# BuTTerK3ks/AA-RMVSNet

Hardware: AMD Instinct MI355X
Metric: depth-hypotheses/sec (ref-views x H x W x D / s) (higher is better)
Workload: dtype fp32-class split-fp16 (3 products: cells, deconvs, omega conv on f16 MFMA, lo*lo dropped, fp32 accumulate; fp32 elsewhere); 1 GPU; dtu_eval_1600x1184_n7_d512; ref_views_per_gpu=1, views=7, H=1184, W=1600, D=512, global_batch=1, parallelism=ref-view shard x1

## Files before the change

aa-rmvsnet_amd/csrc/warp_cost.hip:

```cpp
#include <hip/hip_runtime.h>

#include <cfloat>
#include <climits>
#include <cstdlib>
#include <cstring>

#include "device_common.h"

namespace aarmvs {

__device__ __forceinline__ void sample_pos(const float* __restrict__ m, float depth, float x,
                                           float y, int H, int W, float& ix, float& iy) {
  float p[3];
#pragma unroll
  for (int k = 0; k < 3; ++k) {
    const float rx = __fadd_rn(__fadd_rn(__fmul_rn(m[4 * k + 0], x), __fmul_rn(m[4 * k + 1], y)),
                               m[4 * k + 2]);
    p[k] = __fadd_rn(__fmul_rn(rx, depth), m[4 * k + 3]);
  }
  float z = p[2];
  if (z == 0.0f) z = __fadd_rn(z, 1e-4f);
  const float px = __fdiv_rn(p[0], z), py = __fdiv_rn(p[1], z);
  const float gx = __fsub_rn(__fdiv_rn(px, (float)(W - 1) * 0.5f), 1.0f);
  const float gy = __fsub_rn(__fdiv_rn(py, (float)(H - 1) * 0.5f), 1.0f);
// ... 238 lines not shown
__device__ __forceinline__ void gn_relu4(const float (&x)[4], const GnStat& s, const float* gw,
                                         const float* gb, bool relu, float (&y)[4]) {
#pragma unroll
  for (int c = 0; c < 4; ++c) {
    const float sc = s.rstd * gw[c];
    const float sh = gb[c] - s.mean * sc;
    const float v = x[c] * sc + sh;
    y[c] = relu ? fmaxf(v, 0.0f) : v;
  }
}

__device__ __forceinline__ void conv1x1_4(const float (&x)[4], const float* w, const float* bias,
                                          float (&y)[4]) {
#pragma unroll
  for (int co = 0; co < 4; ++co) {
    float s = 0.f;
#pragma unroll
    for (int ci = 0; ci < 4; ++ci) s = fmaf(w[co * 4 + ci], x[ci], s);
    y[co] = s + bias[co];
  }
}

__device__ __forceinline__ float omega_weight(const float4 q, const GnStat* gs, const OmegaP& o) {
  const float t[4] = {q.x, q.y, q.z, q.w};
  float aa[4], t2[4], bb[4], t3[4], g3[4];
  gn_relu4(t, gs[0], o.g0w, o.g0b, true, aa);
  conv1x1_4(aa, o.w1, o.b1, t2);
  gn_relu4(t2, gs[1], o.g1w, o.g1b, true, bb);
  conv1x1_4(bb, o.w2, o.b2, t3);
  gn_relu4(t3, gs[2], o.g2w, o.g2b, false, g3);
  float s = 0.f;
#pragma unroll
  for (int c = 0; c < 4; ++c) s = fmaf(o.wo[c], fmaxf(g3[c] + aa[c], 0.0f), s);
  return sigmoidf_(s + o.bo);
}

__device__ __forceinline__ size_t st_index(int b, int v, int k, int nsrc) {
  return (((size_t)b * nsrc + v) * 3 + k) * kSlots * 2;
}

constexpr int kTileW = 32, kTileH = 16, kTileThreads = kTileW * kTileH;
constexpr int kTileWaves = kTileThreads / 64;

__device__ __forceinline__ int xcd_tile(int bid, int nb) {
  const int q8 = nb >> 3, r8 = nb & 7, xcd = bid & 7;
  return (xcd < r8 ? xcd * (q8 + 1) : r8 * (q8 + 1) + (xcd - r8) * q8) + (bid >> 3);
}

struct TapF {
  float xf, yf;
  float wt[4];
};

__device__ __forceinline__ TapF tap_f(const float* __restrict__ m, float dep, int x, int y, int H,
                                      int W) {
  float ix, iy;
  sample_pos(m, dep, (float)x, (float)y, H, W, ix, iy);
  TapF t;
  t.xf = floorf(ix);
  t.yf = floorf(iy);
  const float wx = __fsub_rn(ix, t.xf), wy = __fsub_rn(iy, t.yf);
  const float ex = __fsub_rn(1.0f, wx), sy = __fsub_rn(1.0f, wy);
  t.wt[0] = __fmul_rn(sy, ex);
  t.wt[1] = __fmul_rn(sy, wx);
  t.wt[2] = __fmul_rn(wy, ex);
  t.wt[3] = __fmul_rn(wy, wx);
  return t;
}

__device__ __forceinline__ void box_extend(const TapF& t, int H, int W, int& lx, int& ly, int& hx,
                                           int& hy) {
  if (!(t.xf == t.xf) || !(t.yf == t.yf)) return;
  const float xl = fmaxf(t.xf, 0.f), xh = fminf(t.xf + 1.f, (float)(W - 1));
  const float yl = fmaxf(t.yf, 0.f), yh = fminf(t.yf + 1.f, (float)(H - 1));
  if (xl <= xh && yl <= yh) {
    lx = min(lx, (int)xl);
    hx = max(hx, (int)xh);
    ly = min(ly, (int)yl);
    hy = max(hy, (int)yh);
  }
}

struct Box {
  int x0, y0, nx, ny;
};

template <int NW = kTileWaves>
__device__ __forceinline__ Box box_reduce(int lx, int ly, int hx, int hy, int (*red)[4]) {
  const int lane = threadIdx.x & 63, wave = threadIdx.x >> 6;
  auto mn = [](int a, int b) { return min(a, b); };
  auto mx = [](int a, int b) { return max(a, b); };
  lx = wave_reduce_i32(lx, INT_MAX, mn);
  ly = wave_reduce_i32(ly, INT_MAX, mn);
  hx = wave_reduce_i32(hx, INT_MIN, mx);
  hy = wave_reduce_i32(hy, INT_MIN, mx);
  if (lane == 0) {
    red[wave][0] = lx;
    red[wave][1] = ly;
    red[wave][2] = hx;
    red[wave][3] = hy;
  }
  __syncthreads();
#pragma unroll
  for (int w = 0; w < NW; ++w) {
    lx = min(lx, red[w][0]);
    ly = min(ly, red[w][1]);
    hx = max(hx, red[w][2]);
    hy = max(hy, red[w][3]);
  }
  Box bx;
  bx.x0 = __builtin_amdgcn_readfirstlane(lx);
  bx.y0 = __builtin_amdgcn_readfirstlane(ly);
  bx.nx = __builtin_amdgcn_readfirstlane(hx >= lx ? hx - lx + 1 : 0);
  bx.ny = __builtin_amdgcn_readfirstlane(hy >= ly ? hy - ly + 1 : 0);
  return bx;
}

__device__ __forceinline__ uint32_t box_magic(int nx) {
  return nx > 1 ? 0xFFFFFFFFu / (uint32_t)nx + 1u : 0u;
}
__device__ __forceinline__ int box_row(int p, int nx, uint32_t mg) {
  return nx > 1 ? (int)__umulhi((uint32_t)p, mg) : p;
}

struct TapP {
  uint32_t pix[4];
  float wt[4];
};

__device__ __forceinline__ TapP tap_p(const TapF& t, bool valid, int H, int W, bool lds,
                                      const Box& bx, uint32_t zpix) {
  TapP o;
#pragma unroll
  for (int k = 0; k < 4; ++k) {
    o.wt[k] = t.wt[k];
    const float xf = t.xf + (float)(k & 1), yf = t.yf + (float)(k >> 1);
    const bool ok = valid && (xf > -1.0f) && (xf < (float)W) && (yf > -1.0f) && (yf < (float)H);
    const int xi = ok ? (int)xf : bx.x0, yi = ok ? (int)yf : bx.y0;
    const uint32_t p = lds ? __umul24((uint32_t)(yi - bx.y0), (uint32_t)bx.nx) + (uint32_t)(xi - bx.x0)
                           : __umul24((uint32_t)yi, (uint32_t)W) + (uint32_t)xi;
    o.pix[k] = ok ? p : zpix;
  }
  return o;
}

__device__ __forceinline__ TapP tap_p4(const TapF& t, bool valid, int H, int W, bool lds,
                                      const Box& bx, uint32_t zpix) {
  TapP o;
#pragma unroll
  for (int k = 0; k < 4; ++k) o.wt[k] = t.wt[k];
  const float xf1 = t.xf + 1.0f, yf1 = t.yf + 1.0f;
  const bool cx0 = t.xf > -1.0f && t.xf < (float)W, cx1 = xf1 > -1.0f && xf1 < (float)W;
  const bool cy0 = valid && t.yf > -1.0f && t.yf < (float)H;
  const bool cy1 = valid && yf1 > -1.0f && yf1 < (float)H;
  const int ox = lds ? bx.x0 : 0, oy = lds ? bx.y0 : 0, rs = lds ? bx.nx : W;
  const int p00 = __mul24((int)t.yf - oy, rs) + ((int)t.xf - ox);
  o.pix[0] = cy0 && cx0 ? (uint32_t)p00 : zpix;
  o.pix[1] = cy0 && cx1 ? (uint32_t)(p00 + 1) : zpix;
  o.pix[2] = cy1 && cx0 ? (uint32_t)(p00 + rs) : zpix;
  o.pix[3] = cy1 && cx1 ? (uint32_t)(p00 + rs + 1) : zpix;
  return o;
}

__device__ __forceinline__ float bil1(float v0, float v1, float v2, float v3, const TapP& t) {
  return __fmaf_rn(v3, t.wt[3], __fmaf_rn(v2, t.wt[2], __fmaf_rn(v1, t.wt[1], __fmul_rn(v0, t.wt[0]))));
}

__device__ __forceinline__ float4 bil4(float4 v0, float4 v1, float4 v2, float4 v3, const TapP& t) {
  return make_float4(bil1(v0.x, v1.x, v2.x, v3.x, t), bil1(v0.y, v1.y, v2.y, v3.y, t),
                     bil1(v0.z, v1.z, v2.z, v3.z, t), bil1(v0.w, v1.w, v2.w, v3.w, t));
}

__device__ __forceinline__ float4 sqdiff4(float4 g, float4 r) {
  const float dx = __fsub_rn(g.x, r.x), dy = __fsub_rn(g.y, r.y);
  const float dz = __fsub_rn(g.z, r.z), dw = __fsub_rn(g.w, r.w);
  return make_float4(__fmul_rn(dx, dx), __fmul_rn(dy, dy), __fmul_rn(dz, dz), __fmul_rn(dw, dw));
}

__device__ __forceinline__ float4 ld_c8(__amdgpu_buffer_rsrc_t r, uint32_t p, int s, int HW) {
  return ld4(r, (uint32_t)(s >> 1) * (uint32_t)HW * 32u + p * 32u + 16u * (uint32_t)(s & 1));
}

__device__ __forceinline__ float swap_pair(float v) {
  return __int_as_float(__builtin_amdgcn_mov_dpp(__float_as_int(v), 0xB1, 0xF, 0xF, false));
}
__device__ __forceinline__ void sample_pos_pair(const float* __restrict__ m, float depth, float x,
                                                float y, int H, int W, int h, float& ix,
                                                float& iy) {
  auto row = [&](int k) {
    const float rx = __fadd_rn(__fadd_rn(__fmul_rn(m[4 * k + 0], x), __fmul_rn(m[4 * k + 1], y)),
                               m[4 * k + 2]);
    return __fadd_rn(__fmul_rn(rx, depth), m[4 * k + 3]);
  };
  const float ph = h ? row(1) : row(0);
  float z = row(2);
  if (z == 0.0f) z = __fadd_rn(z, 1e-4f);
  const int dim = h ? H : W;
  const float g = __fsub_rn(__fdiv_rn(__fdiv_rn(ph, z), (float)(dim - 1) * 0.5f), 1.0f);
  const float i = __fmaf_rn(__fadd_rn(g, 1.0f), (float)dim * 0.5f, -0.5f);
  const float o = swap_pair(i);
  ix = h ? o : i;
  iy = h ? i : o;
}

constexpr int kXRows = 4;
template <int XV = 0, int XR = kXRows>
__global__ void __launch_bounds__(2 * XR * kTileW)
__attribute__((amdgpu_waves_per_eu((XV & 8) ? 6 : (XV & 4) ? 5 : 4))) cost_x_kernel(PipeArgs a,
                                                              const float* __restrict__ P,
                                                              const float* __restrict__ Rel) {
  __shared__ GnStat gs[AARMVS_MAX_SRC][3];
  const int tid = threadIdx.x, b = blockIdx.y;
  const int H = a.H, W = a.W, HW = H * W, nsrc = a.nsrc;
  const int seq = xcd_tile(blockIdx.x, gridDim.x);
  const int tile = seq / a.npl, kp = seq - tile * a.npl;
  const int tiles_x = (W + kTileW - 1) / kTileW;
  const int h = tid & 1, q = tid >> 1;
  const int gy = (tile / tiles_x) * XR + q / kTileW, gx = (tile % tiles_x) * kTileW + q % kTileW;
  if (tid < 3 * nsrc) {
    const int v = tid / 3, k = tid % 3;
    gs[v][k] = stat_read(a.st_prev + kp * a.st_kstride + st_index(b, v, k, nsrc), 4.0 * HW);
  }
  __syncthreads();
  if (gy >= H || gx >= W) return;
  const float4* __restrict__ t1p = a.t1_prev + kp * a.t1_kstride;
  float* const omega_out = kp == a.omega_k ? a.omega_out : nullptr;
  OmegaP o;
  load_omega(a, P, o);
  const float dep = a.dvals[b * a.D + a.d_prev + kp];
  const uint32_t fbytes = (uint32_t)((size_t)kC * HW * 4);
  const __amdgpu_buffer_rsrc_t rref = uniform_rsrc(a.ref + (size_t)b * kC * HW, fbytes);
  const size_t p = (size_t)gy * W + gx;
  float4 rf[4];
#pragma unroll
  for (int c = 0; c < 4; ++c) rf[c] = ld_c8(rref, (uint32_t)p, 2 * c + h, HW);
  float acc[16];
#pragma unroll
  for (int j = 0; j < 16; ++j) acc[j] = 0.f;
  float wv[AARMVS_MAX_SRC];
#pragma unroll
  for (int vp = 0; vp < AARMVS_MAX_SRC; vp += 2) {
    if ((XV & 2) && vp < nsrc) {
      const int vm = min(vp + h, nsrc - 1);
      const uint32_t p32 = (uint32_t)p, hw = (uint32_t)HW;
      const float w = omega_weight(
          t1p[(uint32_t)(b * nsrc + vp) * hw + (uint32_t)(vm - vp) * hw + p32], gs[vm], o);
      if (omega_out && vp + h < nsrc)
        omega_out[(uint32_t)(vp * a.B + b) * hw + (uint32_t)(h * a.B) * hw + p32] = w;
      const float ws = swap_pair(w);
      wv[vp] = h ? ws : w;
      if (vp + 1 < AARMVS_MAX_SRC) wv[vp + 1] = h ? w : ws;
    }
  }
  for (int v = 0; v < nsrc; ++v) {
    const float* __restrict__ m = Rel + 12 * (v * a.B + b);
    const __amdgpu_buffer_rsrc_t rsrc = uniform_rsrc(a.src[v] + (size_t)b * kC * HW, fbytes);
    float w;
    if constexpr ((XV & 2) != 0) {
      w = wv[0];
#pragma unroll
      for (int k = 1; k < AARMVS_MAX_SRC; ++k) w = v == k ? wv[k] : w;
    } else {
      w = omega_weight(t1p[((size_t)b * nsrc + v) * HW + p], gs[v], o);
      if (omega_out && h == 0) omega_out[((size_t)v * a.B + b) * HW + p] = w;
    }
    const float wp1 = __fadd_rn(w, 1.0f);
    const Box none{0, 0, 0, 0};
    TapF tf;
    if constexpr ((XV & 1) == 0) {
      tf = tap_f(m, dep, gx, gy, H, W);
    } else {
      float ix, iy;
      sample_pos_pair(m, dep, (float)gx, (float)gy, H, W, h, ix, iy);
      tf.xf = floorf(ix);
      tf.yf = floorf(iy);
      const float wx = __fsub_rn(ix, tf.xf), wy = __fsub_rn(iy, tf.yf);
      const float ex = __fsub_rn(1.0f, wx), sy = __fsub_rn(1.0f, wy);
      tf.wt[0] = __fmul_rn(sy, ex);
      tf.wt[1] = __fmul_rn(sy, wx);
      tf.wt[2] = __fmul_rn(wy, ex);
      tf.wt[3] = __fmul_rn(wy, wx);
    }
    const TapP t = tap_p(tf, true, H, W, false, none, fbytes / 32u);
#pragma unroll
    for (int c = 0; c < 4; ++c) {
      const int s = 2 * c + h;
      const float4 g = bil4(ld_c8(rsrc, t.pix[0], s, HW), ld_c8(rsrc, t.pix[1], s, HW),
                            ld_c8(rsrc, t.pix[2], s, HW), ld_c8(rsrc, t.pix[3], s, HW), t);
      const float4 sq = sqdiff4(g, rf[c]);
      float* ac = &acc[4 * c];
      ac[0] = __fadd_rn(ac[0], __fmul_rn(wp1, sq.x));
      ac[1] = __fadd_rn(ac[1], __fmul_rn(wp1, sq.y));
      ac[2] = __fadd_rn(ac[2], __fmul_rn(wp1, sq.z));
      ac[3] = __fadd_rn(ac[3], __fmul_rn(wp1, sq.w));
    }
  }
  float* xo = a.x + kp * a.x_kstride + ((size_t)b * HW + p) * kC + 4 * h;
#pragma unroll
  for (int c = 0; c < 4; ++c) {
    float r[4];
#pragma unroll
    for (int j = 0; j < 4; ++j) r[j] = -1.0f * __fdiv_rn(acc[4 * c + j], (float)nsrc);
    *reinterpret_cast<float4*>(xo + 8 * c) = make_float4(r[0], r[1], r[2], r[3]);
  }
}

__device__ __forceinline__ uint32_t img_slot(uint32_t p, int h) {
  return p * 8u + ((uint32_t)(h ^ (int)((p >> 3) & 1u)) << 2);
}
__device__ __forceinline__ float4 img_ld(const float* img, uint32_t p, int h) {
  return *reinterpret_cast<const float4*>(img + img_slot(p, h));
}
__device__ __forceinline__ void img_st(float* img, uint32_t p, int h, float4 v) {
  *reinterpret_cast<float4*>(img + img_slot(p, h)) = v;
}
__device__ __forceinline__ int img_half(uint32_t p, int s) { return s ^ (int)((p >> 3) & 1u); }

typedef _Float16 half8 __attribute__((ext_vector_type(8)));
typedef _Float16 half4 __attribute__((ext_vector_type(4)));
typedef _Float16 half2_t __attribute__((ext_vector_type(2)));
typedef float float2_t __attribute__((ext_vector_type(2)));
typedef float floatx4 __attribute__((ext_vector_type(4)));
typedef float floatx16 __attribute__((ext_vector_type(16)));

typedef __attribute__((address_space(3))) void* lds_void_ptr;
__device__ __forceinline__ void dma16(__amdgpu_buffer_rsrc_t r, float* wave_dst, uint32_t off,
                                      uint32_t soff = 0) {
  __builtin_amdgcn_raw_ptr_buffer_load_lds(r, (lds_void_ptr)wave_dst, 16, off, soff, 0, 0);
}
__device__ __forceinline__ uint32_t split_pair(float a, float b, uint32_t& lo_bits) {
  const uint32_t hb = __builtin_bit_cast(uint32_t, __builtin_convertvector((float2_t){a, b}, half2_t));
  float la, lb;
  asm("v_fma_mix_f32 %0, %1, -1.0, %2 op_sel_hi:[1,0,0]" : "=v"(la) : "v"(hb), "v"(a));
  asm("v_fma_mix_f32 %0, %1, -1.0, %2 op_sel:[1,0,0] op_sel_hi:[1,0,0]" : "=v"(lb) : "v"(hb), "v"(b));
  lo_bits = __builtin_bit_cast(uint32_t, __builtin_convertvector((float2_t){la, lb}, half2_t));
  return hb;
}
__device__ __forceinline__ void dma_wait() {
  __builtin_amdgcn_s_waitcnt(0x0F70);
}


constexpr int kMTileH = 16;
template <int TW>
struct OmegaTile {
  static constexpr int NT = kMTileH * TW;
  static constexpr int OUTH = kMTileH - 2, OUTW = TW - 2;
  static constexpr int BOXPX = 2 * NT;
  static int tiles(int H, int W) { return ((W + OUTW - 1) / OUTW) * ((H + OUTH - 1) / OUTH); }
  __device__ static int tiles_d(int H, int W) { return ((W + OUTW - 1) / OUTW) * ((H + OUTH - 1) / OUTH); }
};
#ifndef AARMVS_OMEGA_TW
#define AARMVS_OMEGA_TW 16
#endif
constexpr int kOmegaTW = AARMVS_OMEGA_TW;

template <int CTRL, int ROWS>
__device__ __forceinline__ double dpp_f64_u(double v) {
  const long long b = __double_as_longlong(v);
  const int lo = __builtin_amdgcn_mov_dpp((int)(b & 0xffffffffll), CTRL, ROWS, 0xF, false);
  const int hi = __builtin_amdgcn_mov_dpp((int)(b >> 32), CTRL, ROWS, 0xF, false);
  return __longlong_as_double(((long long)hi << 32) | (unsigned)lo);
}
__device__ __forceinline__ void wave_sum2_d(double& u, double& w) {
  u += dpp_f64_u<0xB1, 0xF>(u);
  w += dpp_f64_u<0xB1, 0xF>(w);
  u += dpp_f64_u<0x4E, 0xF>(u);
  w += dpp_f64_u<0x4E, 0xF>(w);
  u += dpp_f64_u<0x141, 0xF>(u);
  w += dpp_f64_u<0x141, 0xF>(w);
  u += dpp_f64_u<0x140, 0xF>(u);
  w += dpp_f64_u<0x140, 0xF>(w);
  u += dpp_f64_u<0x142, 0xA>(u);
  w += dpp_f64_u<0x142, 0xA>(w);
  u += dpp_f64_u<0x143, 0xC>(u);
  w += dpp_f64_u<0x143, 0xC>(w);
  auto rl = [](double v) {
    const long long b = __double_as_longlong(v);
    const int lo = __builtin_amdgcn_readlane((int)(b & 0xffffffffll), 63);
    const int hi = __builtin_amdgcn_readlane((int)(b >> 32), 63);
    return __longlong_as_double(((long long)hi << 32) | (unsigned)lo);
  };
  u = rl(u);
  w = rl(w);
}

struct OmegaPos {
  int tile, ty, tx, v, kp;
};
template <int NW>
__device__ __forceinline__ void omega_block_sum(const double (*ws)[2], double& s0, double& s1) {
  s0 = 0.0;
  s1 = 0.0;
  for (int w = 0; w < NW; ++w) {
    s0 += ws[w][0];
    s1 += ws[w][1];
  }
}

template <int ABL, int TW, bool BAL, typename PA>
__device__ __forceinline__ void omega_item(PA& a, const float* __restrict__ P,
                                           const float* __restrict__ Rel,
                                           const unsigned* __restrict__ xbound, const OmegaPos ip,
                                           double (*wsum)[OmegaTile<TW>::NT / 64][2], int par,
                                           bool has_prev, const OmegaPos pv) {
  using T = OmegaTile<TW>;
  constexpr int kMThreads = T::NT, kMBoxPx = T::BOXPX, kMOutH = T::OUTH, kMOutW = T::OUTW;
  constexpr int NB = (2 * kMBoxPx + kMThreads - 1) / kMThreads;
  static_assert(TW == 16 || TW == 32, "the row sums shift by DPP along one haloed row");
  constexpr int kRefFl = (kMBoxPx + 1) * 8;
  constexpr int YFL = kRefFl + 2 * kMThreads * 4;
  static_assert(2 * kMThreads * 4 <= YFL, "the row-sum images fit in the box space");
  __shared__ __attribute__((aligned(16))) float smem[YFL];
  float* const box = smem;
  float4* const zms = reinterpret_cast<float4*>(smem);
  float4* const zps = zms + kMThreads;
  __shared__ int red[kMThreads / 64][4];
  int tid;
  asm volatile("v_mov_b32 %0, %1" : "=v"(tid) : "v"((int)threadIdx.x));
  const int lane = tid & 63, wave = tid >> 6;
  const int b = blockIdx.z;
  const int H = a.H, W = a.W, HW = H * W, nsrc = a.nsrc;
  const int v = ip.v, kp = ip.kp;
  const int y0 = ip.ty * kMOutH, x0 = ip.tx * kMOutW;
  const int hy = tid / TW, hx = tid % TW;
  const int gy = y0 - 1 + hy, gx = x0 - 1 + hx;
  const bool in_img = gy >= 0 && gy < H && gx >= 0 && gx < W;
  const bool interior = in_img && hy >= 1 && hy <= kMOutH && hx >= 1 && hx <= kMOutW;
  float* const rimg = smem + kRefFl;

  const float dep = a.dvals[b * a.D + a.d_next + kp];
  const float* __restrict__ m = Rel + 12 * (v * a.B + b);
  const uint32_t fbytes = (uint32_t)((size_t)kC * HW * 4);
  const uint32_t cbytes = (uint32_t)HW * 32u;
  const __amdgpu_buffer_rsrc_t rref = uniform_rsrc(a.ref + (size_t)b * kC * HW, fbytes);
  const __amdgpu_buffer_rsrc_t rsrc = uniform_rsrc(a.src[v] + (size_t)b * kC * HW, fbytes);
  TapF tf{};
  int lx = INT_MAX, ly = INT_MAX, bhx = INT_MIN, bhy = INT_MIN;
  if (in_img) {
    if constexpr ((ABL & 16) != 0) {
      tf.xf = (float)gx + 0.25f * dep * 1e-3f;
      tf.yf = (float)gy;
      tf.wt[0] = tf.wt[1] = tf.wt[2] = tf.wt[3] = 0.25f;
      tf.xf = floorf(tf.xf);
    } else {
      tf = tap_f(m, dep, gx, gy, H, W);
    }
    box_extend(tf, H, W, lx, ly, bhx, bhy);
  }
  const Box bx = box_reduce<kMThreads / 64>(lx, ly, bhx, bhy, red);
  if (tid < 8) box[kMBoxPx * 8 + tid] = 0.f;
  if (has_prev && tid == 0) {
    double s0, s1;
    omega_block_sum<kMThreads / 64>(wsum[par ^ 1], s0, s1);
    if (!(ABL & 64)) part_put(a, pv.kp, b, pv.v, pv.tile, s0, s1);
  }
  const bool lds = bx.nx * bx.ny <= min(kMBoxPx, a.box_cap);
  const uint32_t zp = lds ? (uint32_t)kMBoxPx : fbytes / 32u;
  TapP tp = tap_p4(tf, in_img, H, W, lds, bx, zp);
  const int items = lds ? bx.nx * bx.ny * 2 : 0;
  const uint32_t mg = box_magic(bx.nx);
  uint32_t boff[NB];
#pragma unroll
  for (int j = 0; j < NB; ++j) {
    const int i = tid + j * kMThreads, p = i >> 1, r = box_row(p, bx.nx, mg);
    const uint32_t gp = __umul24((uint32_t)(bx.y0 + r), (uint32_t)W) + (uint32_t)bx.x0 +
                        ((uint32_t)p - __umul24((uint32_t)r, (uint32_t)bx.nx));
    boff[j] = gp * 32u + 16u * (uint32_t)img_half((uint32_t)p, i & 1);
  }
  const uint32_t rpix = in_img ? (uint32_t)(gy * W + gx) * 32u : fbytes;
  const int wave_s = __builtin_amdgcn_readfirstlane(wave);
  auto stage = [&](int c) {
    const uint32_t cb = (uint32_t)c * cbytes;
#pragma unroll
    for (int j = 0; j < NB; ++j)
      if (!(ABL & 2) && tid + j * kMThreads < items)
        dma16(rsrc, box + (j * kMThreads + wave_s * 64) * 4, boff[j], cb);
    if (!(ABL & 8)) {
      dma16(rref, rimg + (wave_s * 64) * 4, rpix, cb);
      dma16(rref, rimg + (kMThreads + wave_s * 64) * 4, rpix + 16u, cb);
    }
  };
  int e = 0;
  {
    const float bound = __uint_as_float(*xbound);
    if (bound > 0.0f) {
      const int k = ilogbf(bound);
      e = k >= 134 ? 120 : (k < -100 ? -114 : k - 14);
      e += e & 1;
    }
  }
  const float dsc = ldexpf(1.0f, -(e / 2));
#pragma unroll
  for (int k = 0; k < 4; ++k) tp.wt[k] = __fmul_rn(tp.wt[k], dsc);
  const float* __restrict__ w0t = P + a.off_ow0t;
  const half8* __restrict__ owm = reinterpret_cast<const half8*>(P + a.off_owm);
  floatx16 acc0, acc1;
  if constexpr ((ABL & 1) != 0) {
#pragma unroll
    for (int r = 0; r < 16; ++r) acc0[r] = acc1[r] = 0.f;
  }
  float o4[4] = {0.f, 0.f, 0.f, 0.f};

  stage(0);
  dma_wait();
  __syncthreads();
#pragma unroll 1
  for (int c = 0; c < 4; ++c) {
    const float* const bx_c = box;
    float4 g0, g1;
    if (ABL & 4) {
      g0 = g1 = make_float4(tp.wt[0], tp.wt[1], tp.wt[2], tp.wt[3]);
    } else if (lds) {
      g0 = bil4(img_ld(bx_c, tp.pix[0], 0), img_ld(bx_c, tp.pix[1], 0), img_ld(bx_c, tp.pix[2], 0),
                img_ld(bx_c, tp.pix[3], 0), tp);
      g1 = bil4(img_ld(bx_c, tp.pix[0], 1), img_ld(bx_c, tp.pix[1], 1), img_ld(bx_c, tp.pix[2], 1),
                img_ld(bx_c, tp.pix[3], 1), tp);
    } else {
      g0 = bil4(ld_c8(rsrc, tp.pix[0], 2 * c, HW), ld_c8(rsrc, tp.pix[1], 2 * c, HW),
                ld_c8(rsrc, tp.pix[2], 2 * c, HW), ld_c8(rsrc, tp.pix[3], 2 * c, HW), tp);
      g1 = bil4(ld_c8(rsrc, tp.pix[0], 2 * c + 1, HW), ld_c8(rsrc, tp.pix[1], 2 * c + 1, HW),
                ld_c8(rsrc, tp.pix[2], 2 * c + 1, HW), ld_c8(rsrc, tp.pix[3], 2 * c + 1, HW), tp);
    }
    const float4 rf0 = *reinterpret_cast<const float4*>(rimg + tid * 4);
    const float4 rf1 = *reinterpret_cast<const float4*>(rimg + (kMThreads + tid) * 4);
    auto dsq = [&](float g, float r) {
      const float dd = __fmaf_rn(r, -dsc, g);
      return __fmul_rn(dd, dd);
    };
    const float sq[8] = {dsq(g0.x, rf0.x), dsq(g0.y, rf0.y), dsq(g0.z, rf0.z), dsq(g0.w, rf0.w),
                         dsq(g1.x, rf1.x), dsq(g1.y, rf1.y), dsq(g1.z, rf1.z), dsq(g1.w, rf1.w)};
    half8 Bd, Bl, Bl2;
    if constexpr ((ABL & 128) == 0) {
      Bd = owm[(c * 3 + 0) * 64 + lane];
      Bl = owm[(c * 3 + 1) * 64 + lane];
      Bl2 = owm[(c * 3 + 2) * 64 + lane];
    }
    __syncthreads();
    if (c < 3) stage(c + 1);
    {
      const float* wt = w0t + (4 * kC + 8 * c) * 4;
#pragma unroll
      for (int j = 0; j < 8; ++j)
#pragma unroll
        for (int co = 0; co < 4; ++co) o4[co] = fmaf(sq[j], wt[j * 4 + co], o4[co]);
    }
    uint32_t hw[4], lw[4];
#pragma unroll
    for (int i = 0; i < 4; ++i) hw[i] = split_pair(sq[2 * i], sq[2 * i + 1], lw[i]);
#pragma unroll
    for (int i = 0; i < 4; ++i) {
      const auto r = __builtin_amdgcn_permlane32_swap(hw[i], lw[i], false, false);
      hw[i] = r[0];
      lw[i] = r[1];
    }
    if (BAL && (c & 1)) {
#pragma unroll
      for (int i = 0; i < 4; ++i) {
        hw[i] ^= 0x80008000u;
        lw[i] ^= 0x80008000u;
      }
    }
    if (BAL && c > 0) {
#pragma unroll
      for (int r = 0; r < 16; ++r) {
        acc0[r] = -acc0[r];
        acc1[r] = -acc1[r];
      }
    }
    const half8 A0 = __builtin_bit_cast(half8, u32x4{hw[0], hw[1], hw[2], hw[3]});
    const half8 A1 = __builtin_bit_cast(half8, u32x4{lw[0], lw[1], lw[2], lw[3]});
    if constexpr ((ABL & 128) != 0) {
      Bd = A1;
      Bl = A0;
      Bl2 = A1;
    }
    if (!(ABL & 1)) {
      if (c == 0) {
        const floatx16 z = {};
        acc0 = __builtin_amdgcn_mfma_f32_32x32x16_f16(Bd, A0, z, 0, 0, 0);
        acc1 = __builtin_amdgcn_mfma_f32_32x32x16_f16(Bd, A1, z, 0, 0, 0);
      } else {
        acc0 = __builtin_amdgcn_mfma_f32_32x32x16_f16(Bd, A0, acc0, 0, 0, 0);
        acc1 = __builtin_amdgcn_mfma_f32_32x32x16_f16(Bd, A1, acc1, 0, 0, 0);
      }
      acc0 = __builtin_amdgcn_mfma_f32_32x32x16_f16(Bl, A0, acc0, 0, 0, 0);
      acc1 = __builtin_amdgcn_mfma_f32_32x32x16_f16(Bl, A1, acc1, 0, 0, 0);
      acc0 = __builtin_amdgcn_mfma_f32_32x32x16_f16(Bl2, A0, acc0, 0, 0, 0);
      acc1 = __builtin_amdgcn_mfma_f32_32x32x16_f16(Bl2, A1, acc1, 0, 0, 0);
    } else {
      acc0[0] += (float)A0[0] + (float)Bd[1];
      acc1[0] += (float)A1[0] + (float)Bl[1];
    }
    if (c < 3) {
      dma_wait();
      __syncthreads();
    }
  }
  static constexpr int kShr = TW == 16 ? 0x111 : 0x138, kShl = TW == 16 ? 0x101 : 0x130;
  auto shr1 = [](float x) {
    return __int_as_float(__builtin_amdgcn_update_dpp(0, __float_as_int(x), kShr, 0xF, 0xF, true));
  };
  auto shl1 = [](float x) {
    return __int_as_float(__builtin_amdgcn_update_dpp(0, __float_as_int(x), kShl, 0xF, 0xF, true));
  };
  float zmr[4], zpr[4], z0[4];
#pragma unroll
  for (int co = 0; co < 4; ++co) {
    const float r0 = (shr1(acc0[co]) + acc0[4 + co]) + shl1(acc0[8 + co]);
    const float r1 = (shr1(acc1[co]) + acc1[4 + co]) + shl1(acc1[8 + co]);
    const auto zz = __builtin_amdgcn_permlane32_swap(__float_as_uint(r0), __float_as_uint(r1), false, false);
    zmr[co] = __uint_as_float(zz[0]);
    zpr[co] = __uint_as_float(zz[1]);
    const auto t35 = __builtin_amdgcn_permlane32_swap(__float_as_uint(acc0[12 + co]),
                                                      __float_as_uint(acc1[12 + co]), false, false);
    z0[co] = shr1(__uint_as_float(t35[0])) + shl1(__uint_as_float(t35[1]));
  }
  if constexpr ((ABL & 32) == 0) {
    zms[tid] = make_float4(zmr[0], zmr[1], zmr[2], zmr[3]);
    zps[tid] = make_float4(zpr[0], zpr[1], zpr[2], zpr[3]);
  }
  __syncthreads();
  double ps = 0.0, pss = 0.0;
  if (interior) {
    float g4[4];
    if constexpr ((ABL & 32) != 0) {
#pragma unroll
      for (int co = 0; co < 4; ++co) g4[co] = (zmr[co] + z0[co]) + zpr[co];
    } else {
      const float4 up = zms[tid - TW], dn = zps[tid + TW];
      g4[0] = (up.x + z0[0]) + dn.x;
      g4[1] = (up.y + z0[1]) + dn.y;
      g4[2] = (up.z + z0[2]) + dn.z;
      g4[3] = (up.w + z0[3]) + dn.w;
    }
    if (BAL) {
#pragma unroll
      for (int co = 0; co < 4; ++co) g4[co] = -g4[co];
    }
    const float pe = ldexpf(1.0f, e);
    const float isc = P[a.off_owm_scale] * pe;
    const float* __restrict__ b0 = P + a.off_ob0;
    float4 out;
    out.x = fmaf(g4[0], isc, o4[0] * pe) + b0[0];
    out.y = fmaf(g4[1], isc, o4[1] * pe) + b0[1];
    out.z = fmaf(g4[2], isc, o4[2] * pe) + b0[2];
    out.w = fmaf(g4[3], isc, o4[3] * pe) + b0[3];
    a.t1_next[kp * a.t1_kstride + ((size_t)b * nsrc + v) * HW + gy * W + gx] = out;
    ps = ((double)out.x + (double)out.y) + ((double)out.z + (double)out.w);
    pss = ((double)out.x * out.x + (double)out.y * out.y) + ((double)out.z * out.z + (double)out.w * out.w);
  }
  wave_sum2_d(ps, pss);
  if (lane == 0) {
    wsum[par][wave][0] = ps;
    wsum[par][wave][1] = pss;
  }
}

#ifndef AARMVS_OMEGA_WAVES
#define AARMVS_OMEGA_WAVES 4
#endif
template <int ABL = 0, int TW = kOmegaTW, bool BAL = false>
__global__ void __launch_bounds__(OmegaTile<TW>::NT) __attribute__((amdgpu_waves_per_eu(AARMVS_OMEGA_WAVES)))
omega_mfma_kernel(PipeArgs a, const float* __restrict__ P, const float* __restrict__ Rel,
                  const unsigned* __restrict__ xbound) {
  if (blockDim.x != OmegaTile<TW>::NT) return;
  const int ipb = a.omega_ipb > 1 ? a.omega_ipb : 1;
  const int npl = a.npl, nsrc = a.nsrc;
  const int tiles_x = (a.W + OmegaTile<TW>::OUTW - 1) / OmegaTile<TW>::OUTW;
  const int total = OmegaTile<TW>::tiles_d(a.H, a.W) * nsrc * npl;
  const int seq0 = xcd_tile(blockIdx.x, gridDim.x) * ipb;
  OmegaPos ip;
  ip.tile = seq0 / (nsrc * npl);
  {
    const int vk = seq0 - ip.tile * (nsrc * npl);
    ip.v = vk / npl;
    ip.kp = vk - ip.v * npl;
    ip.ty = ip.tile / tiles_x;
    ip.tx = ip.tile - ip.ty * tiles_x;
  }
  constexpr int NW = OmegaTile<TW>::NT / 64;
  __shared__ double wsum[2][NW][2];
  OmegaPos pv = ip;
  int it = 0;
#pragma unroll 1
  for (; it < ipb; ++it) {
    if (seq0 + it >= total) break;
    if (it) {
      pv = ip;
      if (++ip.kp == npl) {
        ip.kp = 0;
        if (++ip.v == nsrc) {
          ip.v = 0;
          ++ip.tile;
          if (++ip.tx == tiles_x) {
            ip.tx = 0;
            ++ip.ty;
          }
        }
      }
    }
    uint32_t z;
    asm volatile("s_mov_b32 %0, 0" : "=s"(z));
    typedef const __attribute__((address_space(4))) PipeArgs KPipeArgs;
    KPipeArgs& ka = *(KPipeArgs*)((const __attribute__((address_space(4))) char*)&a + z);
    omega_item<ABL, TW, BAL>(ka, P, Rel, xbound, ip, wsum, it & 1, it > 0, pv);
  }
  if (it > 0) {
    __syncthreads();
    if (threadIdx.x == 0) {
      double s0, s1;
      omega_block_sum<NW>(wsum[(it - 1) & 1], s0, s1);
      if (!(ABL & 64)) part_put(a, ip.kp, (int)blockIdx.z, ip.v, ip.tile, s0, s1);
    }
  }
}

template <int STAGE>
__global__ void __launch_bounds__(256) omega_stats_kernel(PipeArgs a,
                                                          const float* __restrict__ P) {
  __shared__ double red[2 * 4];
  __shared__ GnStat gs[2];
  const int v = blockIdx.y, b = blockIdx.z / a.npl, kp = blockIdx.z - b * a.npl;
  const int HW = a.H * a.W;
  double* const st = a.st_next + kp * a.st_kstride;
  if (threadIdx.x < STAGE)
    gs[threadIdx.x] = stat_read(st + st_index(b, v, threadIdx.x, a.nsrc), 4.0 * HW);
  __syncthreads();
  OmegaP o;
  load_omega(a, P, o);
  const float4* t1 = a.t1_next + kp * a.t1_kstride + ((size_t)b * a.nsrc + v) * HW;
  double part[2] = {0.0, 0.0};
  const int gstride = gridDim.x * blockDim.x;
  for (int p0 = blockIdx.x * blockDim.x + threadIdx.x; p0 < HW; p0 += 4 * gstride) {
    float4 qs[4];
#pragma unroll
    for (int u = 0; u < 4; ++u) {
      const int p = p0 + u * gstride;
      qs[u] = p < HW ? t1[p] : make_float4(0.f, 0.f, 0.f, 0.f);
    }
#pragma unroll
    for (int u = 0; u < 4; ++u) {
    if (p0 + u * gstride >= HW) break;
    const float4 q = qs[u];
    const float t[4] = {q.x, q.y, q.z, q.w};
    float aa[4], t2[4];
    gn_relu4(t, gs[0], o.g0w, o.g0b, true, aa);
    conv1x1_4(aa, o.w1, o.b1, t2);
    float r[4];
    if constexpr (STAGE == 1) {
#pragma unroll
      for (int c = 0; c < 4; ++c) r[c] = t2[c];
    } else {
      float bb[4];
      gn_relu4(t2, gs[1], o.g1w, o.g1b, true, bb);
      conv1x1_4(bb, o.w2, o.b2, r);
    }
    part[0] += ((double)r[0] + (double)r[1]) + ((double)r[2] + (double)r[3]);
    part[1] += ((double)r[0] * r[0] + (double)r[1] * r[1]) + ((double)r[2] * r[2] + (double)r[3] * r[3]);
    }
  }
  block_sum_d<2>(part, red);
  if (threadIdx.x == 0) part_put(a, kp, b, v, blockIdx.x, part[0], part[1]);
}

__global__ void __launch_bounds__(256) stat_reduce_kernel(PipeArgs a, int stage) {
  __shared__ double red[2][256];
  const int g = blockIdx.x, v = g % a.nsrc, b = (g / a.nsrc) % a.B, kp = g / (a.nsrc * a.B);
  const double* pp = a.part + 2 * (size_t)g * a.part_n;
  double s = 0.0, ss = 0.0;
  for (int i = threadIdx.x; i < a.part_n; i += 256) {
    s += pp[2 * i];
    ss += pp[2 * i + 1];
  }
  red[0][threadIdx.x] = s;
  red[1][threadIdx.x] = ss;
  __syncthreads();
  for (int o = 128; o > 0; o >>= 1) {
    if (threadIdx.x < o) {
      red[0][threadIdx.x] += red[0][threadIdx.x + o];
      red[1][threadIdx.x] += red[1][threadIdx.x + o];
    }
    __syncthreads();
  }
  if (threadIdx.x == 0) {
    double* st = a.st_next + kp * a.st_kstride + st_index(b, v, stage, a.nsrc);
    st[0] = red[0][0];
    st[1] = red[1][0];
  }
}

static PipeArgs pipe_args(const CostArgs& ca, const SweepGeom& g, const Workspace& ws) {
  const ParamLayout& L = param_layout();
  PipeArgs a{};
  a.ref = ca.ref;
  for (int v = 0; v < AARMVS_MAX_SRC; ++v) a.src[v] = v < g.nsrc ? ca.src[v] : nullptr;
  a.rel = ca.rel;
  a.dvals = ca.depth_values;
  a.D = g.D;
  a.params = ca.params;
  a.x = ws.x;
  a.B = g.B;
  a.H = g.H;
  a.W = g.W;
  a.nsrc = g.nsrc;
  a.box_cap = INT_MAX;
  a.npl = 1;
  a.omega_k = 0;
  a.off_ow0 = L.pk_off[P_OW0];
  a.off_ow0t = L.ow0t_off;
  a.off_owb_scale = L.owb_scale_off;
  a.off_owm = L.owm_off;
  a.off_owm_scale = L.owb_scale_off;
  a.off_ob0 = L.pk_off[P_OB0];
  a.off_og0w = L.pk_off[P_OG0W];
  a.off_og0b = L.pk_off[P_OG0B];
  a.off_ow1 = L.pk_off[P_OW1];
  a.off_ob1 = L.pk_off[P_OB1];
  a.off_og1w = L.pk_off[P_OG1W];
  a.off_og1b = L.pk_off[P_OG1B];
  a.off_ow2 = L.pk_off[P_OW2];
  a.off_ob2 = L.pk_off[P_OB2];
  a.off_og2w = L.pk_off[P_OG2W];
  a.off_og2b = L.pk_off[P_OG2B];
  a.off_owo = L.pk_off[P_OWO];
  a.off_obo = L.pk_off[P_OBO];
  return a;
}

static int pipe_box_cap() {
  const char* s = std::getenv("AARMVS_PIPE_BOX_CAP");
  return (s && *s) ? std::max(4, std::atoi(s)) : INT_MAX;
}

static int omega_ipb(int items, int cu_count) {
  const char* s = std::getenv("AARMVS_OMEGA_IPB");
  if (s && *s) return std::max(1, std::min(8, std::atoi(s)));
  int ipb = 8;
  while (ipb > 1 && (items + ipb - 1) / ipb < 8 * std::max(1, cu_count)) ipb >>= 1;
  return ipb;
}

static PipeArgs pipe_args_c8(const CostArgs& ca, const SweepGeom& g, const Workspace& ws) {
  PipeArgs a = pipe_args(ca, g, ws);
  a.ref = ws.feat8[0];
  for (int v = 0; v < g.nsrc; ++v) a.src[v] = ws.feat8[1 + v];
  a.box_cap = pipe_box_cap();
  return a;
}

static void group_strides(PipeArgs& a, const Workspace& ws, int n) {
  a.npl = n;
  a.t1_kstride = ws.t1_plane;
  a.st_kstride = ws.omega_stats_bytes / sizeof(double);
  a.x_kstride = ws.x_plane;
}

hipError_t launch_cost_x_group(const CostArgs& ca, const SweepGeom& g, const Workspace& ws, int d0,
                               int n, float* x0, float* omega_out, int omega_k, hipStream_t s) {
  PipeArgs a = pipe_args_c8(ca, g, ws);
  group_strides(a, ws, n);
  a.d_prev = d0;
  a.d_next = -1;
  a.x = x0;
  a.t1_prev = reinterpret_cast<const float4*>(ws.t1);
  a.st_prev = ws.omega_stats;
  a.omega_out = omega_out;
  a.omega_k = omega_out ? omega_k : -1;
  const int ntiles = ((g.W + kTileW - 1) / kTileW) * ((g.H + kXRows - 1) / kXRows);
  ProfScope ps(s, K_COST_X);
  hipLaunchKernelGGL(cost_x_kernel<2>, dim3(ntiles * n, g.B), dim3(2 * kXRows * kTileW), 0, s, a,
                     a.params, a.rel);
  return hipGetLastError();
}

hipError_t launch_omega_group(const CostArgs& ca, const SweepGeom& g, const Workspace& ws, int d0,
                              int n, hipStream_t s, bool balanced) {
  PipeArgs a = pipe_args_c8(ca, g, ws);
  group_strides(a, ws, n);
  a.d_prev = -1;
  a.d_next = d0;
  a.t1_next = reinterpret_cast<float4*>(ws.t1);
  a.st_next = ws.omega_stats;
  a.part = ws.omega_part;
  hipError_t e;
  const int nred = n * g.B * g.nsrc;
  if ((e = hipMemsetAsync(ws.omega_stats, 0, (size_t)n * ws.omega_stats_bytes, s)) != hipSuccess)
    return e;
  {
    const int ntiles = OmegaTile<kOmegaTW>::tiles(g.H, g.W);
    ProfScope ps(s, K_OMEGA_CONV);
    a.part_n = ntiles;
    a.omega_ipb = omega_ipb(ntiles * g.nsrc * n * g.B, g.cu_count);
    const int nblk = (ntiles * g.nsrc * n + a.omega_ipb - 1) / a.omega_ipb;
    if (balanced)
      hipLaunchKernelGGL((omega_mfma_kernel<0, kOmegaTW, true>), dim3(nblk, 1, g.B),
                         dim3(OmegaTile<kOmegaTW>::NT), 0, s, a, a.params, a.rel, ws.xbound);
    else
      hipLaunchKernelGGL((omega_mfma_kernel<0, kOmegaTW>), dim3(nblk, 1, g.B),
                         dim3(OmegaTile<kOmegaTW>::NT), 0, s, a, a.params, a.rel, ws.xbound);
    if ((e = hipGetLastError()) != hipSuccess) return e;
  }
  {
    ProfScope ps(s, K_STAT_REDUCE);
    hipLaunchKernelGGL(stat_reduce_kernel, dim3(nred), dim3(256), 0, s, a, 0);
  }
  if ((e = hipGetLastError()) != hipSuccess) return e;
  const int HW = g.H * g.W;
  const int pblk =
      std::max(1, std::min((HW + 1023) / 1024, 8 * g.cu_count / std::max(1, g.B * g.nsrc) + 1));
  a.part_n = pblk;
  {
    ProfScope ps(s, K_OMEGA1);
    hipLaunchKernelGGL(omega_stats_kernel<1>, dim3(pblk, g.nsrc, g.B * n), dim3(256), 0, s, a,
                       a.params);
  }
  if ((e = hipGetLastError()) != hipSuccess) return e;
  {
    ProfScope ps(s, K_STAT_REDUCE);
    hipLaunchKernelGGL(stat_reduce_kernel, dim3(nred), dim3(256), 0, s, a, 1);
  }
  if ((e = hipGetLastError()) != hipSuccess) return e;
  {
    ProfScope ps(s, K_OMEGA2);
    hipLaunchKernelGGL(omega_stats_kernel<2>, dim3(pblk, g.nsrc, g.B * n), dim3(256), 0, s, a,
                       a.params);
  }
  if ((e = hipGetLastError()) != hipSuccess) return e;
  {
    ProfScope ps(s, K_STAT_REDUCE);
    hipLaunchKernelGGL(stat_reduce_kernel, dim3(nred), dim3(256), 0, s, a, 2);
  }
  return hipGetLastError();
}

__global__ void __launch_bounds__(256) nchw_to_c8_kernel(const float* __restrict__ src,
                                                         float* __restrict__ dst, int HW,
                                                         unsigned* __restrict__ xbound) {
  __shared__ float t[kC][65];
  __shared__ float wmax[4];
  const int b = blockIdx.y, p0 = blockIdx.x * 64;
  const float* s = src + (size_t)b * kC * HW;
  float4* d = reinterpret_cast<float4*>(dst + (size_t)b * kC * HW);
  const int px = threadIdx.x & 63;
  float mx = 0.f;
#pragma unroll
  for (int j = 0; j < 8; ++j) {
    const int c = (threadIdx.x >> 6) + 4 * j;
    const float v = p0 + px < HW ? s[(size_t)c * HW + p0 + px] : 0.f;
    t[c][px] = v;
    const float av = fabsf(v);
    mx = (av > mx || av != av) ? av : mx;
  }
  if (xbound) {
#pragma unroll
    for (int o = 32; o > 0; o >>= 1) {
      const float q = __shfl_xor(mx, o, 64);
      mx = (q > mx || q != q) ? q : mx;
    }
    if ((threadIdx.x & 63) == 0) wmax[threadIdx.x >> 6] = mx;
  }
  __syncthreads();
  if (xbound && threadIdx.x == 0) {
    float m = 0.f;
    for (int w = 0; w < 4; ++w) m = (wmax[w] > m || wmax[w] != wmax[w]) ? wmax[w] : m;
    const float bound = 8.0f * m * m;
    const unsigned bits = __float_as_uint(bound != bound ? INFINITY : bound);
    if (bits > __hip_atomic_load(xbound, __ATOMIC_RELAXED, __HIP_MEMORY_SCOPE_AGENT))
      atomicMax(xbound, bits);
  }
#pragma unroll
  for (int j = 0; j < 2; ++j) {
    const int idx = threadIdx.x + 256 * j, ch = idx >> 7, q = (idx & 127) >> 1, h = idx & 1;
    const int c0 = 8 * ch + 4 * h;
    if (p0 + q < HW)
      d[((size_t)ch * HW + p0 + q) * 2 + h] =
          make_float4(t[c0][q], t[c0 + 1][q], t[c0 + 2][q], t[c0 + 3][q]);
  }
}

hipError_t launch_to_c8(const float* src, float* dst, int B, int HW, hipStream_t s,
                        unsigned* xbound) {
  ProfScope ps(s, K_TO_C8);
  hipLaunchKernelGGL(nchw_to_c8_kernel, dim3((HW + 63) / 64, B), dim3(256), 0, s, src, dst, HW,
                     xbound);
  return hipGetLastError();
}

}


namespace aarmvs {

struct OmegaChain {
  float t[4], v1[4], aa[4], t2[4], v2[4], bb[4], t3[4], g3[4], s3[4], w;
};
__device__ __forceinline__ void omega_chain(const float4 q, const GnStat* gs, const OmegaP& o,
                                            OmegaChain& c) {
  c.t[0] = q.x;
  c.t[1] = q.y;
  c.t[2] = q.z;
  c.t[3] = q.w;
#pragma unroll
  for (int i = 0; i < 4; ++i) {
    const float sc = gs[0].rstd * o.g0w[i];
    const float sh = o.g0b[i] - gs[0].mean * sc;
    c.v1[i] = c.t[i] * sc + sh;
    c.aa[i] = fmaxf(c.v1[i], 0.0f);
  }
  conv1x1_4(c.aa, o.w1, o.b1, c.t2);
#pragma unroll
  for (int i = 0; i < 4; ++i) {
    const float sc = gs[1].rstd * o.g1w[i];
    const float sh = o.g1b[i] - gs[1].mean * sc;
    c.v2[i] = c.t2[i] * sc + sh;
    c.bb[i] = fmaxf(c.v2[i], 0.0f);
  }
  conv1x1_4(c.bb, o.w2, o.b2, c.t3);
#pragma unroll
  for (int i = 0; i < 4; ++i) {
    const float sc = gs[2].rstd * o.g2w[i];
    const float sh = o.g2b[i] - gs[2].mean * sc;
    c.g3[i] = c.t3[i] * sc + sh;
  }
  float s = 0.f;
#pragma unroll
  for (int i = 0; i < 4; ++i) {
    c.s3[i] = c.g3[i] + c.aa[i];
    s = fmaf(o.wo[i], fmaxf(c.s3[i], 0.0f), s);
  }
  c.w = sigmoidf_(s + o.bo);
}

struct CbwArgs {
  PipeArgs p;
  const float* gx;
  float* go;
  float* wo;
  float4* gt1;
  const double* gsum;
  double* part;
  unsigned* gmax;
  int d0, pblk;
};

__device__ __forceinline__ void wave_absmax_bits(float m, unsigned* dst) {
  const int b = wave_reduce_i32(__float_as_int(m != m ? INFINITY : m), 0,
                                [](int x, int y) { return x > y ? x : y; });
  if ((threadIdx.x & 63) == 0 && (unsigned)b > __hip_atomic_load(dst, __ATOMIC_RELAXED, __HIP_MEMORY_SCOPE_AGENT))
    atomicMax(dst, (unsigned)b);
}

template <int STAGE>
__global__ void __launch_bounds__(256) cbw_chain_kernel(CbwArgs a, const float* __restrict__ P,
                                                        const float* __restrict__ Rel) {
  constexpr int NCOL = STAGE == 1 ? 15 : STAGE == 4 ? 4 : 30;
  __shared__ double red[NCOL * 4];
  __shared__ GnStat gs[3];
  __shared__ float gm[3][2];
  const PipeArgs& pa = a.p;
  const int v = blockIdx.y, bk = blockIdx.z, b = bk % pa.B, k = bk / pa.B;
  const int H = pa.H, W = pa.W, HW = H * W, nsrc = pa.nsrc;
  const size_t kbv = ((size_t)k * pa.B + b) * nsrc + v;
  if (threadIdx.x < 3)
    gs[threadIdx.x] = stat_read(pa.st_prev + k * pa.st_kstride + st_index(b, v, threadIdx.x, nsrc), 4.0 * HW);
  if (threadIdx.x >= 32 && threadIdx.x < 38) {
    const int i = threadIdx.x - 32;
    const int st = i >> 1;
    gm[st][i & 1] = (float)(a.gsum[kbv * 6 + 2 * st + (i & 1)] / (4.0 * HW));
  }
  __syncthreads();
  OmegaP o;
  load_omega(pa, P, o);
  double s[NCOL];
#pragma unroll
  for (int i = 0; i < NCOL; ++i) s[i] = 0.0;
  const float* m = Rel + 12 * (v * pa.B + b);
  const float dep = pa.dvals[b * pa.D + a.d0 + k];
  const uint32_t fbytes = (uint32_t)((size_t)kC * HW * 4);
  const __amdgpu_buffer_rsrc_t rref = uniform_rsrc(pa.ref + (size_t)b * kC * HW, fbytes);
  const __amdgpu_buffer_rsrc_t rsrc = uniform_rsrc(pa.src[v] + (size_t)b * kC * HW, fbytes);
  const float4* t1p = pa.t1_prev + k * pa.t1_kstride + ((size_t)b * nsrc + v) * HW;
  float* gop = a.go + kbv * HW;
  float amax = 0.f;
  for (int p = blockIdx.x * 256 + threadIdx.x; p < HW; p += gridDim.x * 256) {
    OmegaChain c;
    omega_chain(t1p[p], gs, o, c);
    float g_o;
    if constexpr (STAGE == 1) {
      const int x = p % W, y = p / W;
      const TapF tf = tap_f(m, dep, x, y, H, W);
      const Box none{0, 0, 0, 0};
      const TapP t = tap_p(tf, true, H, W, false, none, fbytes / 32u);
      const float* gxp = a.gx + (((size_t)k * pa.B + b) * HW + p) * kC;
      float dw = 0.f;
#pragma unroll
      for (int sl = 0; sl < 8; ++sl) {
        const float4 g = bil4(ld_c8(rsrc, t.pix[0], sl, HW), ld_c8(rsrc, t.pix[1], sl, HW),
                              ld_c8(rsrc, t.pix[2], sl, HW), ld_c8(rsrc, t.pix[3], sl, HW), t);
        const float4 sq = sqdiff4(g, ld_c8(rref, (uint32_t)p, sl, HW));
        const float4 gg = *reinterpret_cast<const float4*>(gxp + 4 * sl);
        dw += gg.x * sq.x + gg.y * sq.y + gg.z * sq.z + gg.w * sq.w;
        amax = fmaxf(amax, fmaxf(fmaxf(fabsf(gg.x), fabsf(gg.y)), fmaxf(fabsf(gg.z), fabsf(gg.w))));
      }
      dw = -dw / (float)nsrc;
      g_o = dw * c.w * (1.0f - c.w);
      gop[p] = g_o;
      a.wo[kbv * HW + p] = c.w;
    } else {
      g_o = gop[p];
    }
    float g_r[4];
#pragma unroll
    for (int i = 0; i < 4; ++i) g_r[i] = c.s3[i] > 0.f ? o.wo[i] * g_o : 0.f;
    float xh3[4];
#pragma unroll
    for (int i = 0; i < 4; ++i) xh3[i] = (c.t3[i] - gs[2].mean) * gs[2].rstd;
    if constexpr (STAGE == 1) {
#pragma unroll
      for (int i = 0; i < 4; ++i) {
        const float gx3 = g_r[i] * o.g2w[i];
        s[0] += gx3;
        s[1] += gx3 * xh3[i];
        s[2 + i] += g_o * fmaxf(c.s3[i], 0.0f);
        s[7 + i] += g_r[i] * xh3[i];
        s[11 + i] += g_r[i];
      }
      s[6] += g_o;
      continue;
    }
    float g_t3[4];
#pragma unroll
    for (int i = 0; i < 4; ++i) g_t3[i] = gs[2].rstd * (g_r[i] * o.g2w[i] - gm[2][0] - xh3[i] * gm[2][1]);
    float g_n2[4], xh2[4];
#pragma unroll
    for (int ci = 0; ci < 4; ++ci) {
      float ga = 0.f;
#pragma unroll
      for (int co = 0; co < 4; ++co) ga = fmaf(o.w2[co * 4 + ci], g_t3[co], ga);
      g_n2[ci] = c.v2[ci] > 0.f ? ga : 0.f;
      xh2[ci] = (c.t2[ci] - gs[1].mean) * gs[1].rstd;
    }
    if constexpr (STAGE == 2) {
#pragma unroll
      for (int i = 0; i < 4; ++i) {
        const float gx2 = g_n2[i] * o.g1w[i];
        s[0] += gx2;
        s[1] += gx2 * xh2[i];
#pragma unroll
        for (int j = 0; j < 4; ++j) s[2 + i * 4 + j] += g_t3[i] * c.bb[j];
        s[18 + i] += g_t3[i];
        s[22 + i] += g_n2[i] * xh2[i];
        s[26 + i] += g_n2[i];
      }
      continue;
    }
    float g_t2[4];
#pragma unroll
    for (int i = 0; i < 4; ++i) g_t2[i] = gs[1].rstd * (g_n2[i] * o.g1w[i] - gm[1][0] - xh2[i] * gm[1][1]);
    float g_n1[4], xh1[4];
#pragma unroll
    for (int ci = 0; ci < 4; ++ci) {
      float ga = g_r[ci];
#pragma unroll
      for (int co = 0; co < 4; ++co) ga = fmaf(o.w1[co * 4 + ci], g_t2[co], ga);
      g_n1[ci] = c.v1[ci] > 0.f ? ga : 0.f;
      xh1[ci] = (c.t[ci] - gs[0].mean) * gs[0].rstd;
    }
    if constexpr (STAGE == 3) {
#pragma unroll
      for (int i = 0; i < 4; ++i) {
        const float gx1 = g_n1[i] * o.g0w[i];
        s[0] += gx1;
        s[1] += gx1 * xh1[i];
#pragma unroll
// ... 701 lines not shown
```

Before: 1.198 billion depth-hypotheses/s.

## Process multiple depth planes per cost_x block, reusing bilinear source taps

Adds a cost_x kernel in which each block handles PP depth planes, with PP set to 2 by default. It loads the reference features once and, for each source view, reloads the 16 bilinear tap vectors only when the sample position moves between consecutive planes. The aim is to cut repeated gathers of reference and source features and to reduce the number of blocks launched. In exchange each thread holds more registers (PP accumulators of 16 floats), which can lower occupancy, and the launch hints for waves per EU change accordingly.

New measurement: 1.223 billion depth-hypotheses/s (median of 6 runs). +2.0%, better.

```diff
diff --git a/aa-rmvsnet_amd/csrc/warp_cost.hip b/aa-rmvsnet_amd/csrc/warp_cost.hip
--- a/aa-rmvsnet_amd/csrc/warp_cost.hip
+++ b/aa-rmvsnet_amd/csrc/warp_cost.hip
@@ -564,6 +564,129 @@
 #pragma unroll
     for (int j = 0; j < 4; ++j) r[j] = -1.0f * __fdiv_rn(acc[4 * c + j], (float)nsrc);
     *reinterpret_cast<float4*>(xo + 8 * c) = make_float4(r[0], r[1], r[2], r[3]);
+  }
+}
+
+template <int XR, int PP>
+__global__ void __launch_bounds__(2 * XR * kTileW)
+__attribute__((amdgpu_waves_per_eu(PP >= 4 ? 2 : 3))) cost_x_planes_kernel(
+    PipeArgs a, const float* __restrict__ P, const float* __restrict__ Rel) {
+  static_assert(3 * AARMVS_MAX_SRC * PP <= 2 * XR * kTileW, "one statistic per thread");
+  __shared__ GnStat gs[PP][AARMVS_MAX_SRC][3];
+  __shared__ float wl[PP][AARMVS_MAX_SRC][XR * kTileW];
+  const int tid = threadIdx.x, b = blockIdx.y;
+  const int H = a.H, W = a.W, HW = H * W, nsrc = a.nsrc;
+  const int seq = xcd_tile(blockIdx.x, gridDim.x);
+  const int nkb = (a.npl + PP - 1) / PP;
+  const int tile = seq / nkb, kp0 = (seq - tile * nkb) * PP;
+  const int np = min(PP, a.npl - kp0);
+  const int tiles_x = (W + kTileW - 1) / kTileW;
+  const int h = tid & 1, q = tid >> 1;
+  const int gy = (tile / tiles_x) * XR + q / kTileW, gx = (tile % tiles_x) * kTileW + q % kTileW;
+  if (tid < 3 * nsrc * np) {
+    const int j = tid / (3 * nsrc), r = tid - j * 3 * nsrc;
+    const int v = r / 3, k = r % 3;
+    gs[j][v][k] =
+        stat_read(a.st_prev + (kp0 + j) * a.st_kstride + st_index(b, v, k, nsrc), 4.0 * HW);
+  }
+  __syncthreads();
+  if (gy >= H || gx >= W) return;
+  const uint32_t fbytes = (uint32_t)((size_t)kC * HW * 4);
+  const size_t p = (size_t)gy * W + gx;
+  float dep[PP];
+  {
+    OmegaP o;
+    load_omega(a, P, o);
+#pragma unroll
+    for (int j = 0; j < PP; ++j) {
+      if (j >= np) continue;
+      const int kp = kp0 + j;
+      dep[j] = a.dvals[b * a.D + a.d_prev + kp];
+      const float4* __restrict__ t1p = a.t1_prev + kp * a.t1_kstride;
+      float* const omega_out = kp == a.omega_k ? a.omega_out : nullptr;
+      for (int vp = 0; vp < nsrc; vp += 2) {
+        const int vm = min(vp + h, nsrc - 1);
+        const uint32_t p32 = (uint32_t)p, hw = (uint32_t)HW;
+        const float w = omega_weight(
+            t1p[(uint32_t)(b * nsrc + vp) * hw + (uint32_t)(vm - vp) * hw + p32], gs[j][vm], o);
+        if (vp + h < nsrc) {
+          if (omega_out) omega_out[(uint32_t)(vp * a.B + b) * hw + (uint32_t)(h * a.B) * hw + p32] = w;
+          wl[j][vp + h][q] = w;
+        }
+      }
+    }
+  }
+  __builtin_amdgcn_wave_barrier();
+  const __amdgpu_buffer_rsrc_t rref = uniform_rsrc(a.ref + (size_t)b * kC * HW, fbytes);
+  float4 rf[4];
+#pragma unroll
+  for (int c = 0; c < 4; ++c) rf[c] = ld_c8(rref, (uint32_t)p, 2 * c + h, HW);
+  float acc[PP][16];
+#pragma unroll
+  for (int j = 0; j < PP; ++j)
+#pragma unroll
+    for (int i = 0; i < 16; ++i) acc[j][i] = 0.f;
+  for (int v = 0; v < nsrc; ++v) {
+    const float* __restrict__ m = Rel + 12 * (v * a.B + b);
+    const __amdgpu_buffer_rsrc_t rsrc = uniform_rsrc(a.src[v] + (size_t)b * kC * HW, fbytes);
+    float4 R[16];
+    const Box none{0, 0, 0, 0};
+    TapP tp[PP];
+    bool moved[PP];
+    float wp1[PP];
+    {
+      const TapF tf = tap_f(m, dep[0], gx, gy, H, W);
+      tp[0] = tap_p(tf, true, H, W, false, none, fbytes / 32u);
+#pragma unroll
+      for (int c = 0; c < 4; ++c)
+#pragma unroll
+        for (int k = 0; k < 4; ++k) R[4 * c + k] = ld_c8(rsrc, tp[0].pix[k], 2 * c + h, HW);
+      wp1[0] = __fadd_rn(wl[0][v][q], 1.0f);
+      float pxf = tf.xf, pyf = tf.yf;
+#pragma unroll
+      for (int j = 1; j < PP; ++j) {
+        if (j >= np) continue;
+        const TapF tj = tap_f(m, dep[j], gx, gy, H, W);
+        tp[j] = tap_p(tj, true, H, W, false, none, fbytes / 32u);
+        moved[j] = !(tj.xf == pxf && tj.yf == pyf);
+        pxf = tj.xf;
+        pyf = tj.yf;
+        wp1[j] = __fadd_rn(wl[j][v][q], 1.0f);
+      }
+    }
+#pragma unroll
+    for (int j = 0; j < PP; ++j) {
+      if (j >= np) continue;
+      const TapP& t = tp[j];
+      if (j > 0 && moved[j]) {
+#pragma unroll
+        for (int c = 0; c < 4; ++c)
+#pragma unroll
+          for (int k = 0; k < 4; ++k) R[4 * c + k] = ld_c8(rsrc, t.pix[k], 2 * c + h, HW);
+      }
+#pragma unroll
+      for (int c = 0; c < 4; ++c) {
+        const float4 g = bil4(R[4 * c], R[4 * c + 1], R[4 * c + 2], R[4 * c + 3], t);
+        const float4 sq = sqdiff4(g, rf[c]);
+        float* ac = &acc[j][4 * c];
+        ac[0] = __fadd_rn(ac[0], __fmul_rn(wp1[j], sq.x));
+        ac[1] = __fadd_rn(ac[1], __fmul_rn(wp1[j], sq.y));
+        ac[2] = __fadd_rn(ac[2], __fmul_rn(wp1[j], sq.z));
+        ac[3] = __fadd_rn(ac[3], __fmul_rn(wp1[j], sq.w));
+      }
+    }
+  }
+#pragma unroll
+  for (int j = 0; j < PP; ++j) {
+    if (j >= np) continue;
+    float* xo = a.x + (kp0 + j) * a.x_kstride + ((size_t)b * HW + p) * kC + 4 * h;
+#pragma unroll
+    for (int c = 0; c < 4; ++c) {
+      float r[4];
+#pragma unroll
+      for (int i = 0; i < 4; ++i) r[i] = -1.0f * __fdiv_rn(acc[j][4 * c + i], (float)nsrc);
+      *reinterpret_cast<float4*>(xo + 8 * c) = make_float4(r[0], r[1], r[2], r[3]);
+    }
   }
 }
 
@@ -1103,6 +1226,13 @@
   return ipb;
 }
 
+constexpr int kCostXPlanes = 2;
+static int cost_x_planes() {
+  const char* s = std::getenv("AARMVS_COST_X_PLANES");
+  const int v = (s && *s) ? std::atoi(s) : kCostXPlanes;
+  return v >= 4 ? 4 : v >= 2 ? 2 : 1;
+}
+
 static PipeArgs pipe_args_c8(const CostArgs& ca, const SweepGeom& g, const Workspace& ws) {
   PipeArgs a = pipe_args(ca, g, ws);
   a.ref = ws.feat8[0];
@@ -1130,9 +1260,15 @@
   a.omega_out = omega_out;
   a.omega_k = omega_out ? omega_k : -1;
   const int ntiles = ((g.W + kTileW - 1) / kTileW) * ((g.H + kXRows - 1) / kXRows);
+  const int pp = cost_x_planes();
+  const dim3 grid(ntiles * ((n + pp - 1) / pp), g.B), block(2 * kXRows * kTileW);
   ProfScope ps(s, K_COST_X);
-  hipLaunchKernelGGL(cost_x_kernel<2>, dim3(ntiles * n, g.B), dim3(2 * kXRows * kTileW), 0, s, a,
-                     a.params, a.rel);
+  if (pp == 4)
+    hipLaunchKernelGGL((cost_x_planes_kernel<kXRows, 4>), grid, block, 0, s, a, a.params, a.rel);
+  else if (pp == 2)
+    hipLaunchKernelGGL((cost_x_planes_kernel<kXRows, 2>), grid, block, 0, s, a, a.params, a.rel);
+  else
+    hipLaunchKernelGGL(cost_x_kernel<2>, grid, block, 0, s, a, a.params, a.rel);
   return hipGetLastError();
 }
 
```
